# risc0/zeth

Hardware: AMD Instinct MI355X
Metric: segments/sec (higher is better)
Workload: dtype u32

## Files before the change

### zeth_amd/csrc/common.h

```cpp
#pragma once
#include <hip/hip_runtime.h>

#include <atomic>
#include <cstdarg>
#include <cstdio>
#include <cstdlib>
#include <cstring>
#include <map>
#include <string>
#include <vector>

#include "../../include/zkhal.h"
#include "fp.h"
#include "noise.h"

namespace zkh {

inline const char* make_err(const char* fmt, ...) {
    char buf[512];
    va_list ap;
    va_start(ap, fmt);
    vsnprintf(buf, sizeof buf, fmt, ap);
    va_end(ap);
    return strdup(buf);
}
#define ZKH_HIP(expr)                                                                               \
    do {                                                                                            \
        hipError_t _e = (expr);                                                                     \
        if (_e != hipSuccess) return zkh::make_err("%s failed: %s (%s:%d)", #expr, hipGetErrorString(_e), __FILE__, __LINE__); \
    } while (0)
#define ZKH_TRY(expr)                    \
    do {                                 \
        const char* _err = (expr);       \
        if (_err) return _err;           \
    } while (0)
#define ZKH_REQUIRE(cond, ...)                         \
    do {                                               \
        if (!(cond)) return zkh::make_err(__VA_ARGS__); \
    } while (0)

constexpr int ZKH_P2_PTAB = 414;
constexpr int TW_BITS = 12;
constexpr int TW_SIZE = 1 << TW_BITS;
constexpr int TW_HI_BITS = 14;
constexpr int TW_HI_SIZE = 1 << TW_HI_BITS;
constexpr int MAX_LOG_N = TW_BITS + TW_HI_BITS;
constexpr int LDS_TW_LOG = 12;

struct DeviceTables {
    uint32_t* rc;
    uint32_t* diag;
    uint32_t* tw_fwd_lo; uint32_t* tw_fwd_hi;
    uint32_t* tw_rev_lo; uint32_t* tw_rev_hi;
    uint32_t* tile_fwd;  uint32_t* tile_rev;
    uint32_t* layer_fwd; uint32_t* layer_rev;
    uint32_t* layer_fwd_lazy;
    uint32_t* shift_lo;  uint32_t* shift_hi;
};

struct ProfAgg { uint64_t calls = 0; double ms = 0; double bytes = 0; };
struct ProfPending { std::string name; hipEvent_t a, b; double bytes; };

}

struct zkh_alloc_t {
    void* ptr;
    size_t bytes;
    std::atomic<int> refs;
    bool owned;
    zkh_ctx* ctx;
    zkh_alloc_t(void* p, size_t b, int r, bool o, zkh_ctx* c) : ptr(p), bytes(b), refs(r), owned(o), ctx(c) {}
};

struct zkh_buf {
    zkh_alloc_t* a;
    size_t off, len;
    std::atomic<int> refs;
    zkh_buf(zkh_alloc_t* al, size_t o, size_t l, int r) : a(al), off(o), len(l), refs(r) {}
    uint32_t* ptr() const { return (uint32_t*)a->ptr + off; }
};

struct zkh_ctx {
    int device;
    hipStream_t stream;
    zkh::DeviceTables tab;
    uint32_t rou_fwd[28], rou_rev[28];
    uint32_t h_rc[24 * 29], h_diag[zkh::ZKH_P2_PTAB];
    std::multimap<size_t, void*> pool;
    size_t pool_bytes = 0, live_bytes = 0, peak_bytes = 0;
// ... 58 lines not shown
```

### zeth_amd/csrc/fp.h

```cpp
#pragma once
#include <stdint.h>

#if defined(__HIPCC__)
#include <hip/hip_runtime.h>
#define ZKH_HD __host__ __device__ __forceinline__
#else
#define ZKH_HD inline
#endif

namespace zkh {

constexpr uint32_t P = 2013265921u;
constexpr uint32_t PINV = 0x88000001u;
constexpr uint32_t NEG_PINV = 0x77ffffffu;
constexpr uint32_t R1 = 268435454u;
constexpr uint32_t R2 = 1172168163u;
constexpr uint32_t INVALID = 0xffffffffu;

struct Fp {
    uint32_t v;
    ZKH_HD Fp() : v(0) {}
    ZKH_HD explicit constexpr Fp(uint32_t raw, int) : v(raw) {}
    static ZKH_HD Fp raw(uint32_t r) { return Fp(r, 0); }
    static ZKH_HD Fp one() { return Fp(R1, 0); }
// ... 21 lines not shown
    return borrow ? t + P : t;
#endif
}
ZKH_HD uint32_t mont_reduce(uint64_t t) {
    const uint32_t m = (uint32_t)t * NEG_PINV;
    const uint64_t s = t + (uint64_t)m * P;
    return reduce_once((uint32_t)(s >> 32));
}
ZKH_HD int64_t mad_i64(int32_t a, int32_t b, int64_t acc) {
#if defined(__HIP_DEVICE_COMPILE__)
    int64_t d; uint64_t carry;
    asm("v_mad_i64_i32 %0, %1, %2, %3, %4" : "=v"(d), "=s"(carry) : "v"(a), "v"(b), "v"(acc));
    return d;
#else
    return (int64_t)((uint64_t)acc + (uint64_t)((int64_t)a * b));
#endif
}
ZKH_HD int64_t mad_i64_k(int32_t a, int32_t b_uniform, int64_t acc) {
#if defined(__HIP_DEVICE_COMPILE__)
    int64_t d; uint64_t carry;
    asm("v_mad_i64_i32 %0, %1, %2, %3, %4" : "=v"(d), "=s"(carry) : "v"(a), "s"(b_uniform), "v"(acc));
    return d;
#else
    return (int64_t)((uint64_t)acc + (uint64_t)((int64_t)a * b_uniform));
#endif
}
ZKH_HD int64_t mul_i64(int32_t a, int32_t b) {
#if defined(__HIP_DEVICE_COMPILE__)
    int64_t d; uint64_t carry;
    asm("v_mad_i64_i32 %0, %1, %2, %3, 0" : "=v"(d), "=s"(carry) : "v"(a), "v"(b));
    return d;
#else
    return (int64_t)a * b;
#endif
}
ZKH_HD int32_t smont_reduce(int64_t t) {
    const int32_t m = (int32_t)((uint32_t)t * NEG_PINV);
    return (int32_t)(mad_i64_k(m, (int32_t)P, t) >> 32);
}
ZKH_HD int32_t smont(int32_t a, int32_t b) {
    const int64_t t = (int64_t)a * b;
    const int32_t m = (int32_t)((uint32_t)t * NEG_PINV);
    const int64_t s = t + (int64_t)m * (int64_t)P;
    return (int32_t)(s >> 32);
}
ZKH_HD uint32_t canon(int32_t x) { const uint32_t u = (uint32_t)x, v = u + P; return v < u ? v : u; }
ZKH_HD int32_t center(uint32_t x) { return (int32_t)(x - (x > (P - 1) / 2 ? P : 0u)); }
ZKH_HD uint32_t mul_mod(uint32_t a, uint32_t b) { return mont_reduce((uint64_t)a * b); }

ZKH_HD Fp operator+(Fp a, Fp b) { return Fp::raw(add_mod(a.v, b.v)); }
ZKH_HD Fp operator-(Fp a, Fp b) { return Fp::raw(sub_mod(a.v, b.v)); }
ZKH_HD Fp operator*(Fp a, Fp b) { return Fp::raw(mul_mod(a.v, b.v)); }
ZKH_HD Fp operator-(Fp a) { return Fp::raw(a.v ? P - a.v : 0); }
ZKH_HD bool operator==(Fp a, Fp b) { return a.v == b.v; }
ZKH_HD Fp& operator+=(Fp& a, Fp b) { a = a + b; return a; }
ZKH_HD Fp& operator-=(Fp& a, Fp b) { a = a - b; return a; }
ZKH_HD Fp& operator*=(Fp& a, Fp b) { a = a * b; return a; }

ZKH_HD Fp fp_encode(uint32_t x) { return Fp::raw(mul_mod(R2, x % P)); }
ZKH_HD uint32_t fp_decode(Fp a) { return mul_mod(1u, a.v); }
ZKH_HD Fp fp_pow(Fp a, uint64_t e) {
    Fp r = Fp::one();
    while (e) { if (e & 1) r = r * a; a = a * a; e >>= 1; }
    return r;
}
ZKH_HD Fp fp_inv(Fp a) { return fp_pow(a, P - 2); }
// ... 81 lines not shown
```

### zeth_amd/csrc/hal.hip

```cpp
#include <algorithm>

#include "common.h"

#include <sys/random.h>
#include "poseidon2.h"
#include "ntt_lazy.h"
#include "../../include/zkh_poseidon2_consts.h"

using namespace zkh;

extern "C" void zkh_free_error(const char* e) { free((void*)e); }
#if ZKH_P2_CONSTS_ARE_PLACEHOLDER
extern "C" const char* zkh_version(void) { return "zkhal-mi355x 0.2.0 (gfx950; poseidon2_consts=placeholder)"; }
#elif ZKH_P2_CONSTS_ARE_DERIVED
extern "C" const char* zkh_version(void) { return "zkhal-mi355x 0.2.0 (gfx950; poseidon2_consts=derived)"; }
#else
extern "C" const char* zkh_version(void) { return "zkhal-mi355x 0.2.0 (gfx950; poseidon2_consts=upstream)"; }
#endif

namespace zkh {

const char* pool_alloc(zkh_ctx* c, size_t bytes, void** out) {
    bytes = (bytes + 255) & ~(size_t)255;
    if (bytes == 0) bytes = 256;
// ... 135 lines not shown
    if (const char* err = ctx_init_tables(c)) {
        zkh_ctx_destroy(c);
        return err;
    }
    *out = c;
    return nullptr;
}
static const char* ctx_init_tables(zkh_ctx* c) {
    Fp g = fp_encode(137);
    for (int k = 0; k <= 27; k++) {
        Fp w = fp_pow(g, 1ull << (27 - k));
        c->rou_fwd[k] = w.v;
        c->rou_rev[k] = fp_inv(w).v;
    }
    Fp wf = Fp::raw(c->rou_fwd[MAX_LOG_N]), wr = Fp::raw(c->rou_rev[MAX_LOG_N]);
    ZKH_TRY(upload(&c->tab.tw_fwd_lo, powers(wf, TW_SIZE)));
    ZKH_TRY(upload(&c->tab.tw_fwd_hi, powers(fp_pow(wf, TW_SIZE), TW_HI_SIZE)));
    ZKH_TRY(upload(&c->tab.tw_rev_lo, powers(wr, TW_SIZE)));
    ZKH_TRY(upload(&c->tab.tw_rev_hi, powers(fp_pow(wr, TW_SIZE), TW_HI_SIZE)));
    ZKH_TRY(upload(&c->tab.tile_fwd, powers(Fp::raw(c->rou_fwd[LDS_TW_LOG]), 1 << (LDS_TW_LOG - 1))));
    ZKH_TRY(upload(&c->tab.tile_rev, powers(Fp::raw(c->rou_rev[LDS_TW_LOG]), 1 << (LDS_TW_LOG - 1))));
    {
        std::vector<uint32_t> lf(1 << LDS_TW_LOG, R1), lr(1 << LDS_TW_LOG, R1);
        for (int j = 1; j <= LDS_TW_LOG; j++) {
            auto pf = powers(Fp::raw(c->rou_fwd[j]), (size_t)1 << (j - 1)), pr = powers(Fp::raw(c->rou_rev[j]), (size_t)1 << (j - 1));
            for (size_t e = 0; e < pf.size(); e++) { lf[((size_t)1 << (j - 1)) + e] = pf[e]; lr[((size_t)1 << (j - 1)) + e] = pr[e]; }
        }
        ZKH_TRY(upload(&c->tab.layer_fwd, lf));
        ZKH_TRY(upload(&c->tab.layer_rev, lr));
        static_assert(LAZY_TAB_LOG == LDS_TW_LOG, "the lazy table covers the per-layer tables");
        std::vector<uint32_t> lz(LAZY_TAB_WORDS);
        lazy_layer_table(lz.data(), lf.data());
        ZKH_TRY(upload(&c->tab.layer_fwd_lazy, lz));
    }
    Fp three = fp_encode(3);
    ZKH_TRY(upload(&c->tab.shift_lo, powers(three, TW_SIZE)));
    ZKH_TRY(upload(&c->tab.shift_hi, powers(fp_pow(three, TW_SIZE), TW_HI_SIZE)));
    ZKH_TRY(upload(&c->tab.rc, std::vector<uint32_t>(24 * 29)));
    ZKH_TRY(upload(&c->tab.diag, std::vector<uint32_t>(ZKH_P2_PTAB)));
    ZKH_TRY(zkh_poseidon2_set_constants(c, ZKH_P2_ROUND_CONSTANTS, ZKH_P2_M_INT_DIAG));
    ZKH_TRY(ntt_device_init(c));
    ZKH_HIP(hipMalloc((void**)&c->d_fail, 8));
    ZKH_HIP(hipMemsetAsync(c->d_fail, 0, 8, c->stream));
    ZKH_HIP(hipHostMalloc((void**)&c->h_fail, 8, hipHostMallocDefault));
    c->h_fail[0] = c->h_fail[1] = 0;
    return nullptr;
}
extern "C" const char* zkh_ctx_trim(zkh_ctx* c) {
    bind_thread(c);
    ZKH_HIP(hipStreamSynchronize(c->stream));
    for (auto& kv : c->pool) (void)hipFree(kv.second);
    c->pool.clear(); c->pool_bytes = 0;
    return nullptr;
}
extern "C" void zkh_ctx_memory(const zkh_ctx* c, size_t* live, size_t* cached, size_t* peak) {
    if (live) *live = c->live_bytes;
    if (cached) *cached = c->pool_bytes;
    if (peak) *peak = c->peak_bytes;
}
extern "C" void zkh_ctx_destroy(zkh_ctx* c) {
    if (!c) return;
    (void)hipSetDevice(c->device);
    (void)hipStreamSynchronize(c->stream);
    for (auto& kv : c->pool) (void)hipFree(kv.second);
    uint32_t* t[] = {c->tab.rc, c->tab.diag, c->tab.tw_fwd_lo, c->tab.tw_fwd_hi, c->tab.tw_rev_lo, c->tab.tw_rev_hi,
                     c->tab.tile_fwd, c->tab.tile_rev, c->tab.shift_lo, c->tab.shift_hi, c->tab.layer_fwd, c->tab.layer_rev, c->tab.layer_fwd_lazy};
// ... 396 lines not shown
```

### zeth_amd/csrc/ntt.hip

```cpp
#include "common.h"
#include "ntt_lazy.h"

using namespace zkh;

namespace {

constexpr int NTT_THREADS = 256;

struct PassParams {
    const uint32_t* in;
    uint32_t* out;
    size_t in_col_stride;
    size_t out_col_stride;
    uint32_t log_n;
    uint32_t L, R;
    uint32_t log_t;
    uint32_t expand_bits;
    uint32_t first_layer;
    uint32_t twiddle;
    uint32_t scale;
    uint32_t zk_shift;
    const uint32_t* tile_tw;
    const uint32_t* layer_tw;
    const uint32_t* tw_lo;
    const uint32_t* tw_hi;
    const uint32_t* sh_lo;
    const uint32_t* sh_hi;
    uint32_t tiles_per_col;
    uint32_t lazy;
    uint32_t lazy_comp;
    uint32_t shift16[16];
};

template <bool INVERSE>
__global__ __launch_bounds__(NTT_THREADS) void k_ntt_pass(PassParams p) {
    extern __shared__ __attribute__((aligned(16))) uint32_t tile[];
    const uint32_t T = 1u << p.log_t, rows = 1u << p.R, elems = rows << p.log_t;
    const uint32_t tid = threadIdx.x;
    const uint32_t tile_id = xcd_remap(blockIdx.x, p.tiles_per_col);
    const uint32_t col = blockIdx.y;
    const uint32_t ltiles = 1u << (p.L - p.log_t);
    const uint32_t a = tile_id >> (p.L - p.log_t), lt = tile_id & (ltiles - 1);
    const size_t base = ((size_t)a << (p.L + p.R)) + ((size_t)lt << p.log_t);
    const uint32_t l0 = lt << p.log_t;
    const uint32_t* in = p.in + (size_t)col * p.in_col_stride;
    uint32_t* out = p.out + (size_t)col * p.out_col_stride;
    const uint32_t tw_shift = MAX_LOG_N - (p.L + p.R);

    for (uint32_t e = tid; e < elems; e += NTT_THREADS) {
        const uint32_t m = e >> p.log_t, t = e & (T - 1);
        const size_t gi = base + ((size_t)m << p.L) + t;
        uint32_t v = in[gi >> p.expand_bits];
        if (!INVERSE && p.twiddle) {
            const uint32_t r = __brev(m) >> (32 - p.R);
            const uint32_t ex = ((l0 + t) * r) << tw_shift;
            const uint32_t w = mul_mod(p.tw_lo[ex & (TW_SIZE - 1)], p.tw_hi[ex >> TW_BITS]);
            v = mul_mod(v, w);
        }
        tile[e] = v;
    }
    __syncthreads();

    const uint32_t half_elems = elems >> 1;
    if (INVERSE) {
// ... 138 lines not shown
    const uint32_t mid = blockIdx.x;
    const uint32_t rmid = mid_bits ? __brev(mid) >> (32 - mid_bits) : 0;
    if (rmid < mid) return;
    uint32_t* col = io + (size_t)blockIdx.y * col_stride;
    const uint32_t H = 1u << BR_H;
    for (uint32_t e = threadIdx.x; e < H * H; e += blockDim.x) {
        const uint32_t hi = e >> BR_H, lo = e & (H - 1);
        ta[e] = col[((size_t)hi << (log_n - BR_H)) | ((size_t)mid << BR_H) | lo];
        if (rmid != mid) tb[e] = col[((size_t)hi << (log_n - BR_H)) | ((size_t)rmid << BR_H) | lo];
    }
    __syncthreads();
    for (uint32_t e = threadIdx.x; e < H * H; e += blockDim.x) {
        const uint32_t hi2 = e >> BR_H, lo2 = e & (H - 1);
        const uint32_t shi = __brev(lo2) >> (32 - BR_H), slo = __brev(hi2) >> (32 - BR_H);
        const uint32_t src = (shi << BR_H) | slo;
        col[((size_t)hi2 << (log_n - BR_H)) | ((size_t)rmid << BR_H) | lo2] = ta[src];
        if (rmid != mid) col[((size_t)hi2 << (log_n - BR_H)) | ((size_t)mid << BR_H) | lo2] = tb[src];
    }
}
__global__ void k_bit_reverse_small(uint32_t* io, uint32_t log_n, size_t count) {
    size_t g = (size_t)blockIdx.x * blockDim.x + threadIdx.x;
    size_t n = (size_t)1 << log_n;
    if (g >= n * count) return;
    uint32_t i = (uint32_t)(g & (n - 1));
    uint32_t r = log_n ? __brev(i) >> (32 - log_n) : 0;
    if (i < r) {
        uint32_t* col = io + (g - i);
        uint32_t x = col[i], y = col[r];
        col[i] = y; col[r] = x;
    }
}


template <int LOGR, bool INVERSE, bool BASE0, int J_LO, bool LAZY = false>
__device__ __forceinline__ void radix_layers(uint32_t (&v)[1 << LOGR], const uint32_t* __restrict__ ltab,
                                             const uint32_t base_low, const int first_b) {
    constexpr int N = 1 << LOGR;
    if (!INVERSE && LAZY) {
        lazy_layers<LOGR, BASE0, J_LO>(v, ltab, base_low, first_b);
    } else if (INVERSE) {
#pragma unroll
        for (int b = LOGR - 1; b >= 0; b--) {
            const uint32_t* tw = ltab + (1u << (J_LO + b - 1));
#pragma unroll
            for (int kk = 0; kk < (1 << b); kk++) {
                const bool unit = BASE0 && kk == 0;
                const uint32_t w = unit ? 0u : tw[base_low + ((uint32_t)kk << (J_LO - 1))];
#pragma unroll
                for (int hi = 0; hi < (N >> (b + 1)); hi++) {
                    const int k = (hi << (b + 1)) | kk;
                    const uint32_t x = v[k], y = v[k + (1 << b)];
                    v[k] = add_mod(x, y);
                    v[k + (1 << b)] = unit ? sub_mod(x, y) : mul_mod(x - y + P, w);
                }
            }
        }
    } else {
#pragma unroll
        for (int b = 0; b < LOGR; b++) {
            if (b < first_b) continue;
            const uint32_t* tw = ltab + (1u << (J_LO + b - 1));
#pragma unroll
            for (int kk = 0; kk < (1 << b); kk++) {
                const bool unit = BASE0 && kk == 0;
                const uint32_t w = unit ? 0u : tw[base_low + ((uint32_t)kk << (J_LO - 1))];
#pragma unroll
                for (int hi = 0; hi < (N >> (b + 1)); hi++) {
                    const int k = (hi << (b + 1)) | kk;
                    const uint32_t x = v[k], y = unit ? v[k + (1 << b)] : mul_mod(v[k + (1 << b)], w);
                    v[k] = add_mod(x, y);
                    v[k + (1 << b)] = sub_mod(x, y);
                }
            }
        }
    }
// ... 46 lines not shown
        if (p.expand_bits == 0) {
#pragma unroll
            for (int q = 0; q < 4; q++) {
                const uint4 w = ((const uint4*)(in + pos0))[q];
                v[4 * q] = w.x; v[4 * q + 1] = w.y; v[4 * q + 2] = w.z; v[4 * q + 3] = w.w;
            }
        } else if (p.expand_bits == 2) {
            const uint4 w = *(const uint4*)(in + (pos0 >> 2));
            v[0] = v[1] = v[2] = v[3] = w.x; v[4] = v[5] = v[6] = v[7] = w.y;
            v[8] = v[9] = v[10] = v[11] = w.z; v[12] = v[13] = v[14] = v[15] = w.w;
        } else {
#pragma unroll
            for (int k = 0; k < 16; k++) v[k] = in[(pos0 + k) >> p.expand_bits];
        }
        radix_layers<4, false, true, 1, LAZY>(v, ltab, 0, (int)p.expand_bits);
#pragma unroll
        for (int q = 0; q < 4; q++) ((uint4*)lds)[tid * 4 + q] = make_uint4(v[4 * q], v[4 * q + 1], v[4 * q + 2], v[4 * q + 3]);
        __syncthreads();
#pragma unroll
        for (int k = 0; k < 16; k++) v[k] = lds[hi * 256 + k * 16 + low];
        radix_layers<4, false, false, 5, LAZY>(v, ltab, low, 0);
#pragma unroll
        for (int k = 0; k < 16; k++) lds[hi * 256 + k * 16 + low] = v[k];
        __syncthreads();
#pragma unroll
        for (int k = 0; k < 16; k++) v[k] = lds[k * 256 + tid];
        radix_layers<4, false, false, 9, LAZY>(v, ltab, tid, 0);
#pragma unroll
        for (int k = 0; k < 16; k++) out[base + k * 256 + tid] = v[k];
    }
}

template <int RH, bool INVERSE, bool LAZY = false>
__global__ __launch_bounds__(1 << RH) void k_ntt_high(PassParams p) {
    constexpr int LT = 4;
    constexpr uint32_t TW = 1u << LT;
    extern __shared__ __attribute__((aligned(16))) uint32_t lds[];
    const uint32_t tid = threadIdx.x, t = tid & (TW - 1), g = tid >> LT;
    const uint32_t tile_id = xcd_remap(blockIdx.x, p.tiles_per_col), col = blockIdx.y;
    const uint32_t lt_bits = p.L - LT;
    const uint32_t a = tile_id >> lt_bits, lt = tile_id & ((1u << lt_bits) - 1);
    const size_t base = ((size_t)a << (p.L + RH)) + ((size_t)lt << LT);
    const uint32_t lcol = (lt << LT) + t;
    const uint32_t tw_shift = MAX_LOG_N - (p.L + RH);
    const char* in = (const char*)(p.in + (size_t)col * p.in_col_stride + base);
    char* out = (char*)(p.out + (size_t)col * p.out_col_stride + base);
    const uint32_t tb = t * 4u;
#define TILE_IN(row) (*(const uint32_t*)(in + ((((uint32_t)(row)) << (p.L + 2)) + tb)))
#define TILE_OUT(row) (*(uint32_t*)(out + ((((uint32_t)(row)) << (p.L + 2)) + tb)))
    const uint32_t* __restrict__ ltab = p.layer_tw;
    auto tmul = [](uint32_t x, uint32_t y) -> uint32_t {
        return (LAZY && !INVERSE) ? (uint32_t)smont((int32_t)x, (int32_t)y) : mul_mod(x, y);
    };
    auto root = [&](uint32_t e) -> uint32_t {
        const uint32_t ex = e << tw_shift;
        return tmul(p.tw_lo[ex & (TW_SIZE - 1)], p.tw_hi[ex >> TW_BITS]);
    };
    uint32_t tw[16];
    if (RH == 10) {
        uint32_t w0 = root(lcol * (__brev(g) >> 26));
        if (LAZY) w0 = tmul(w0, p.lazy_comp);
        const uint32_t u1 = root(lcol * 64u), v1 = root(lcol * 256u);
        const uint32_t u2 = tmul(u1, u1), u3 = tmul(u2, u1), v2 = tmul(v1, v1), v3 = tmul(v2, v1);
        const uint32_t wi[4] = {w0, tmul(w0, u2), tmul(w0, u1), tmul(w0, u3)};
#pragma unroll
        for (int i = 0; i < 4; i++) {
            tw[4 * i] = wi[i]; tw[4 * i + 1] = tmul(wi[i], v2); tw[4 * i + 2] = tmul(wi[i], v1); tw[4 * i + 3] = tmul(wi[i], v3);
        }
    } else {
        uint32_t w0 = root(lcol * (__brev(g) >> 28));
        if (LAZY) w0 = tmul(w0, p.lazy_comp);
        const uint32_t q1 = root(lcol * 16u);
        uint32_t qp[16];
        qp[0] = w0;
#pragma unroll
        for (int e = 1; e < 16; e++) qp[e] = tmul(qp[e - 1], q1);
#pragma unroll
        for (int k = 0; k < 16; k++) tw[k] = qp[__builtin_bitreverse8((unsigned char)k) >> 4];
    }
    uint32_t v[16];
    if (RH == 10) {
        const uint32_t hi = g >> 2, low = g & 3;
        if (INVERSE) {
#pragma unroll
            for (int k = 0; k < 16; k++) v[k] = TILE_IN(k * 64 + g);
            radix_layers<4, true, false, 7>(v, ltab, g, 0);
#pragma unroll
            for (int k = 0; k < 16; k++) lds[(k * 64 + g) * TW + t] = v[k];
            __syncthreads();
#pragma unroll
            for (int k = 0; k < 16; k++) v[k] = lds[(hi * 64 + k * 4 + low) * TW + t];
            radix_layers<4, true, false, 3>(v, ltab, low, 0);
#pragma unroll
            for (int k = 0; k < 16; k++) lds[(hi * 64 + k * 4 + low) * TW + t] = v[k];
            __syncthreads();
#pragma unroll
            for (int i = 0; i < 4; i++) {
                uint32_t u[4];
                const uint32_t m0 = (g * 4 + i) * 4;
#pragma unroll
                for (int k = 0; k < 4; k++) u[k] = lds[(m0 + k) * TW + t];
                radix_layers<2, true, true, 1>(u, ltab, 0, 0);
#pragma unroll
                for (int k = 0; k < 4; k++) {
                    uint32_t x = mul_mod(u[k], tw[4 * i + k]);
                    if (p.scale) x = mul_mod(x, p.scale);
                    TILE_OUT(m0 + k) = x;
                }
            }
        } else {
#pragma unroll
            for (int i = 0; i < 4; i++) {
                uint32_t u[4];
                const uint32_t m0 = (g * 4 + i) * 4;
#pragma unroll
                for (int k = 0; k < 4; k++) {
                    const uint32_t x = TILE_IN(m0 + k);
                    u[k] = LAZY ? (uint32_t)smont((int32_t)x, (int32_t)tw[4 * i + k]) : mul_mod(x, tw[4 * i + k]);
                }
                radix_layers<2, false, true, 1, LAZY>(u, ltab, 0, 0);
#pragma unroll
                for (int k = 0; k < 4; k++) lds[(m0 + k) * TW + t] = u[k];
            }
            __syncthreads();
#pragma unroll
            for (int k = 0; k < 16; k++) v[k] = lds[(hi * 64 + k * 4 + low) * TW + t];
            radix_layers<4, false, false, 3, LAZY>(v, ltab, low, 0);
#pragma unroll
            for (int k = 0; k < 16; k++) lds[(hi * 64 + k * 4 + low) * TW + t] = v[k];
            __syncthreads();
#pragma unroll
            for (int k = 0; k < 16; k++) v[k] = lds[(k * 64 + g) * TW + t];
            radix_layers<4, false, false, 7, LAZY>(v, ltab, g, 0);
#pragma unroll
            for (int k = 0; k < 16; k++) TILE_OUT(k * 64 + g) = LAZY ? canon((int32_t)v[k]) : v[k];
        }
    } else {
        if (INVERSE) {
#pragma unroll
            for (int k = 0; k < 16; k++) v[k] = TILE_IN(k * 16 + g);
            radix_layers<4, true, false, 5>(v, ltab, g, 0);
#pragma unroll
            for (int k = 0; k < 16; k++) lds[(k * 16 + g) * TW + t] = v[k];
            __syncthreads();
#pragma unroll
            for (int k = 0; k < 16; k++) v[k] = lds[(g * 16 + k) * TW + t];
            radix_layers<4, true, true, 1>(v, ltab, 0, 0);
#pragma unroll
            for (int k = 0; k < 16; k++) {
                uint32_t x = mul_mod(v[k], tw[k]);
                if (p.scale) x = mul_mod(x, p.scale);
                TILE_OUT(g * 16 + k) = x;
            }
        } else {
#pragma unroll
            for (int k = 0; k < 16; k++) {
                const uint32_t x = TILE_IN(g * 16 + k);
                v[k] = LAZY ? (uint32_t)smont((int32_t)x, (int32_t)tw[k]) : mul_mod(x, tw[k]);
            }
            radix_layers<4, false, true, 1, LAZY>(v, ltab, 0, 0);
#pragma unroll
            for (int k = 0; k < 16; k++) lds[(g * 16 + k) * TW + t] = v[k];
            __syncthreads();
#pragma unroll
            for (int k = 0; k < 16; k++) v[k] = lds[(k * 16 + g) * TW + t];
            radix_layers<4, false, false, 5, LAZY>(v, ltab, g, 0);
#pragma unroll
            for (int k = 0; k < 16; k++) TILE_OUT(k * 16 + g) = LAZY ? canon((int32_t)v[k]) : v[k];
        }
    }
}
#undef TILE_IN
#undef TILE_OUT

struct Pass { uint32_t L, R; };
std::vector<Pass> plan_passes(uint32_t log_n) {
    std::vector<Pass> v;
    if (log_n <= 12) { v.push_back({0, log_n}); return v; }
    if (log_n < 18) {
        const uint32_t low = (log_n + 1) / 2;
        v.push_back({0, low});
        v.push_back({low, log_n - low});
        return v;
    }
    const uint32_t rem = log_n - 12;
    v.push_back({0, 12});
    if (rem == 8 || rem == 10 || rem <= 7) v.push_back({12, rem});
    else if (rem == 9) { v.push_back({12, 8}); v.push_back({20, 1}); }
    else if (rem == 11 || rem == 12) { v.push_back({12, 8}); v.push_back({20, rem - 8}); }
    else { v.push_back({12, 10}); v.push_back({22, rem - 10}); }
    return v;
}

const char* run_transform(zkh_ctx* c, bool inverse, const uint32_t* in, size_t in_col_stride, uint32_t* out,
                          size_t out_col_stride, uint32_t log_n, size_t count, uint32_t expand_bits, bool zk, const char* name) {
    ZKH_REQUIRE(log_n <= (uint32_t)MAX_LOG_N, "%s: transform size 2^%u exceeds the supported 2^%d", name, log_n, MAX_LOG_N);
    ZKH_REQUIRE(count <= 65535, "%s: too many columns (%zu)", name, count);
    std::vector<Pass> passes = plan_passes(log_n);
    const size_t n = (size_t)1 << log_n;
    Fp ninv = fp_inv(fp_encode((uint32_t)(n % P)));
    const size_t npass = passes.size();
    const bool lazy = !inverse && npass == 2 && passes[0].R == 12 && (passes[1].R == 8 || passes[1].R == 10) && expand_bits <= 4;
    const uint32_t lazy_reds = lazy ? lazy_reductions(4, expand_bits) + 2 * lazy_reductions(4, 0) + lazy_reductions(passes[1].R, 0) : 0;
    const uint32_t lazy_comp = lazy ? fp_pow(Fp::raw(R2), lazy_reds).v : 0;
    for (size_t pi = 0; pi < npass; pi++) {
        const Pass ps = inverse ? passes[npass - 1 - pi] : passes[pi];
        PassParams p{};
        const bool first = pi == 0, last = pi + 1 == npass;
        p.in = first ? in : out;
        p.in_col_stride = first ? in_col_stride : out_col_stride;
        p.out = out; p.out_col_stride = out_col_stride;
        p.log_n = log_n; p.L = ps.L; p.R = ps.R;
        const bool reg_high = ps.L >= 4 && (ps.R == 8 || ps.R == 10);
        p.log_t = ps.L == 0 ? 0 : (ps.L < 4 ? ps.L : 4);
        if (ps.L != 0 && !reg_high && ps.R < 12) p.log_t = std::max<uint32_t>(p.log_t, std::min<uint32_t>(ps.L, 12 - ps.R));
        while (p.R + p.log_t > 14 && p.log_t > 0) p.log_t--;
        p.expand_bits = (!inverse && first) ? expand_bits : 0;
        p.first_layer = (!inverse && first) ? expand_bits + 1 : 1;
        p.twiddle = ps.L != 0;
        p.scale = (inverse && last) ? ninv.v : 0;
        p.zk_shift = (inverse && last && zk) ? 1 : 0;
        p.lazy = lazy; p.lazy_comp = lazy_comp;
        p.tile_tw = inverse ? c->tab.tile_rev : c->tab.tile_fwd;
        p.layer_tw = inverse ? c->tab.layer_rev : (lazy ? c->tab.layer_fwd_lazy : c->tab.layer_fwd);
        p.tw_lo = inverse ? c->tab.tw_rev_lo : c->tab.tw_fwd_lo;
        p.tw_hi = inverse ? c->tab.tw_rev_hi : c->tab.tw_fwd_hi;
        p.sh_lo = c->tab.shift_lo; p.sh_hi = c->tab.shift_hi;
        if (p.zk_shift && log_n >= 4) {
            const Fp three = fp_encode(3);
            for (uint32_t k = 0; k < 16; k++)
                p.shift16[k] = (ninv * fp_pow(three, (uint64_t)(bitrev32(k) >> 28) << (log_n - 4))).v;
        }
        p.tiles_per_col = (uint32_t)(n >> (p.R + p.log_t));
        const size_t lds = ((size_t)4 << (p.R + p.log_t));
        dim3 grid(p.tiles_per_col, (unsigned)count);
        const double alg_bytes = pi == 0 ? 4.0 * count * (double)(((size_t)1 << log_n) >> expand_bits) + 4.0 * count * (double)n : 0.0;
        const bool scale_here = p.scale != 0;
        const bool k_low = ps.L == 0 && ps.R == 12 && p.expand_bits <= 4;
        const bool k_h10 = !k_low && ps.L >= 4 && p.log_t == 4 && ps.R == 10 && !(scale_here && p.zk_shift);
        const bool k_h8 = !k_low && !k_h10 && ps.L >= 4 && p.log_t == 4 && ps.R == 8 && !(scale_here && p.zk_shift);
        const bool k_top = !k_low && !k_h10 && !k_h8 && ps.L >= 12 && ps.L + ps.R == log_n && ps.R >= 1 && ps.R <= 4 && p.twiddle &&
                           p.expand_bits == 0 && p.first_layer == 1 && !scale_here && !p.zk_shift;
        const std::string pname = std::string(name) + (k_low ? ":k_ntt_low12" : k_h10 ? ":k_ntt_high10" : k_h8 ? ":k_ntt_high8" : k_top ? ":k_ntt_top" : ":k_ntt_pass");
        ProfScope prof(c, pname.c_str(), alg_bytes);
        if (ps.L == 0 && ps.R == 12 && p.expand_bits <= 4) {
            if (inverse) k_ntt_low12<true><<<grid, 256, 0, c->stream>>>(p);
            else if (lazy) k_ntt_low12<false, true><<<grid, 256, 0, c->stream>>>(p);
            else k_ntt_low12<false><<<grid, 256, 0, c->stream>>>(p);
        } else if (ps.L >= 4 && p.log_t == 4 && ps.R == 10 && !(scale_here && p.zk_shift)) {
            if (inverse) k_ntt_high<10, true><<<grid, 1024, lds, c->stream>>>(p);
            else if (lazy) k_ntt_high<10, false, true><<<grid, 1024, lds, c->stream>>>(p);
            else k_ntt_high<10, false><<<grid, 1024, lds, c->stream>>>(p);
        } else if (ps.L >= 4 && p.log_t == 4 && ps.R == 8 && !(scale_here && p.zk_shift)) {
            if (inverse) k_ntt_high<8, true><<<grid, 256, lds, c->stream>>>(p);
            else if (lazy) k_ntt_high<8, false, true><<<grid, 256, lds, c->stream>>>(p);
            else k_ntt_high<8, false><<<grid, 256, lds, c->stream>>>(p);
        } else if (k_top) {
            const dim3 tg((unsigned)(((size_t)1 << ps.L) >> 10), (unsigned)count);
            switch (ps.R * 2 + (inverse ? 1 : 0)) {
            case 2: k_ntt_top<1, false><<<tg, 256, 0, c->stream>>>(p); break;
            case 3: k_ntt_top<1, true><<<tg, 256, 0, c->stream>>>(p); break;
            case 4: k_ntt_top<2, false><<<tg, 256, 0, c->stream>>>(p); break;
            case 5: k_ntt_top<2, true><<<tg, 256, 0, c->stream>>>(p); break;
            case 6: k_ntt_top<3, false><<<tg, 256, 0, c->stream>>>(p); break;
            case 7: k_ntt_top<3, true><<<tg, 256, 0, c->stream>>>(p); break;
            case 8: k_ntt_top<4, false><<<tg, 256, 0, c->stream>>>(p); break;
            default: k_ntt_top<4, true><<<tg, 256, 0, c->stream>>>(p); break;
            }
        } else if (inverse) k_ntt_pass<true><<<grid, NTT_THREADS, lds, c->stream>>>(p);
        else k_ntt_pass<false><<<grid, NTT_THREADS, lds, c->stream>>>(p);
        ZKH_TRY(last_launch_error(name));
    }
    return nullptr;
}

}

const char* zkh::ntt_device_init(zkh_ctx* c) {
    bind_thread(c);
    ZKH_HIP(hipFuncSetAttribute((const void*)k_ntt_high<10, true>, hipFuncAttributeMaxDynamicSharedMemorySize, 65536));
    ZKH_HIP(hipFuncSetAttribute((const void*)k_ntt_high<10, false>, hipFuncAttributeMaxDynamicSharedMemorySize, 65536));
    ZKH_HIP(hipFuncSetAttribute((const void*)k_ntt_high<10, false, true>, hipFuncAttributeMaxDynamicSharedMemorySize, 65536));
    return nullptr;
}

static const char* interpolate_impl(zkh_ctx* c, zkh_buf* io, size_t count, bool zk, const char* name) {
    ZKH_REQUIRE(count && io->len % count == 0, "%s: size %zu not a multiple of count %zu", name, io->len, count);
    const size_t n = io->len / count;
    const uint32_t log_n = log2_ceil(n);
    ZKH_REQUIRE(((size_t)1 << log_n) == n, "%s: column length %zu is not a power of two", name, n);
    return run_transform(c, true, io->ptr(), n, io->ptr(), n, log_n, count, 0, zk, name);
}
extern "C" const char* zkh_batch_interpolate_ntt(zkh_ctx* c, zkh_buf* io, size_t count) {
    return interpolate_impl(c, io, count, false, "batch_interpolate_ntt");
}
extern "C" const char* zkh_batch_interpolate_ntt_zk_shift(zkh_ctx* c, zkh_buf* io, size_t count) {
    return interpolate_impl(c, io, count, true, "batch_interpolate_ntt_zk_shift");
}
extern "C" const char* zkh_batch_interpolate_ntt_from(zkh_ctx* c, zkh_buf* out, const zkh_buf* in, size_t count, int zk_shift) {
    ZKH_REQUIRE(count && in->len % count == 0 && out->len == in->len, "batch_interpolate_ntt_from: shape mismatch");
    const size_t n = in->len / count;
    const uint32_t log_n = log2_ceil(n);
    ZKH_REQUIRE(((size_t)1 << log_n) == n, "batch_interpolate_ntt_from: column length %zu is not a power of two", n);
    return run_transform(c, true, in->ptr(), n, out->ptr(), n, log_n, count, 0, zk_shift != 0, "batch_interpolate_ntt_from");
}
extern "C" const char* zkh_batch_expand_into_evaluate_ntt(zkh_ctx* c, zkh_buf* out, const zkh_buf* in, size_t count,
                                                          size_t expand_bits) {
    ZKH_REQUIRE(count && out->len % count == 0 && in->len % count == 0, "batch_expand_into_evaluate_ntt: sizes not multiples of count");
    const size_t n_out = out->len / count, n_in = in->len / count;
    const uint32_t log_n = log2_ceil(n_out);
    ZKH_REQUIRE(((size_t)1 << log_n) == n_out && (n_in << expand_bits) == n_out,
                "batch_expand_into_evaluate_ntt: out column %zu != in column %zu << %zu", n_out, n_in, expand_bits);
    ZKH_REQUIRE(expand_bits <= log_n, "batch_expand_into_evaluate_ntt: expand_bits too large");
    if (expand_bits == log_n) {
        return make_err("batch_expand_into_evaluate_ntt: expand_bits == log2(size) unsupported");
// ... 28 lines not shown
```

### zeth_amd/csrc/ntt_lazy.h

```cpp
#pragma once
#include "fp.h"

#ifndef ZKH_LAZY_SUM
#define ZKH_LAZY_SUM(t) ((void)0)
#endif

namespace zkh {

constexpr int LAZY_TAB_LOG = 12;
constexpr uint32_t LAZY_TAB_MONT = 1u << LAZY_TAB_LOG;
constexpr uint32_t LAZY_TAB_WORDS = 2u << LAZY_TAB_LOG;

inline void lazy_layer_table(uint32_t* out, const uint32_t* layer_fwd) {
    for (uint32_t i = 0; i < LAZY_TAB_MONT; i++) {
        out[i] = (uint32_t)center(mont_reduce((uint64_t)layer_fwd[i]));
        out[LAZY_TAB_MONT + i] = (uint32_t)center(layer_fwd[i]);
    }
}

template <bool UNIFORM>
ZKH_HD int64_t lazy_mad(int32_t a, int32_t w, int64_t acc) {
    if constexpr (UNIFORM) return mad_i64_k(a, w, acc);
    else return mad_i64(a, w, acc);
}
// ... 35 lines not shown
    constexpr int N = 1 << LOGR;
#pragma unroll
    for (int b = 0; b < LOGR; b += 2) {
        const uint32_t* twa = ltab + (1u << (J_LO + b - 1));
        const uint32_t* twb = ltab + LAZY_TAB_MONT + (1u << (J_LO + b));
        if (b >= first_b) {
#pragma unroll
            for (int kk = 0; kk < (1 << b); kk++) {
                const uint32_t e = base_low + ((uint32_t)kk << (J_LO - 1));
                const int32_t wa = (BASE0 && kk == 0) ? 1 : (int32_t)twa[e];
                const int32_t wb0 = (BASE0 && kk == 0) ? (int32_t)R1 : (int32_t)twb[e];
                const int32_t wb1 = (int32_t)twb[e + ((1u << b) << (J_LO - 1))];
#pragma unroll
                for (int hi = 0; hi < (N >> (b + 2)); hi++) {
                    const int k = (hi << (b + 2)) | kk;
                    lazy_pair<BASE0>(v[k], v[k + (1 << b)], v[k + (2 << b)], v[k + (3 << b)], wa, wb0, wb1);
                }
            }
        } else if (b + 1 >= first_b) {
            const uint32_t* tw1 = ltab + (1u << (J_LO + b));
#pragma unroll
            for (int kk = 0; kk < (2 << b); kk++) {
                const int32_t w = (BASE0 && kk == 0) ? 1 : (int32_t)tw1[base_low + ((uint32_t)kk << (J_LO - 1))];
#pragma unroll
                for (int hi = 0; hi < (N >> (b + 2)); hi++) {
                    const int k = (hi << (b + 2)) | kk;
                    lazy_single<BASE0>(v[k], v[k + (2 << b)], w);
                }
            }
        }
    }
}

}
```

Measured before the change: 44.43.

## Add lazy signed-Montgomery inverse tail for strided high NTT pass

```diff
diff --git a/zeth_amd/csrc/common.h b/zeth_amd/csrc/common.h
--- a/zeth_amd/csrc/common.h
+++ b/zeth_amd/csrc/common.h
@@ -55,6 +55,7 @@
     uint32_t* tile_fwd;  uint32_t* tile_rev;
     uint32_t* layer_fwd; uint32_t* layer_rev;
     uint32_t* layer_fwd_lazy;
+    int32_t lazy_inv_a = 0, lazy_inv_b = 0;
     uint32_t* shift_lo;  uint32_t* shift_hi;
 };
 
diff --git a/zeth_amd/csrc/fp.h b/zeth_amd/csrc/fp.h
--- a/zeth_amd/csrc/fp.h
+++ b/zeth_amd/csrc/fp.h
@@ -77,6 +77,15 @@
     return d;
 #else
     return (int64_t)a * b;
+#endif
+}
+ZKH_HD int64_t mul_i64_k(int32_t a, int32_t b_uniform) {
+#if defined(__HIP_DEVICE_COMPILE__)
+    int64_t d; uint64_t carry;
+    asm("v_mad_i64_i32 %0, %1, %2, %3, 0" : "=v"(d), "=s"(carry) : "v"(a), "s"(b_uniform));
+    return d;
+#else
+    return (int64_t)a * b_uniform;
 #endif
 }
 ZKH_HD int32_t smont_reduce(int64_t t) {
diff --git a/zeth_amd/csrc/hal.hip b/zeth_amd/csrc/hal.hip
--- a/zeth_amd/csrc/hal.hip
+++ b/zeth_amd/csrc/hal.hip
@@ -191,6 +191,8 @@
         std::vector<uint32_t> lz(LAZY_TAB_WORDS);
         lazy_layer_table(lz.data(), lf.data());
         ZKH_TRY(upload(&c->tab.layer_fwd_lazy, lz));
+        ZKH_REQUIRE(lazy_inv_short_pair(fp_decode(Fp::raw(lr[3])), &c->tab.lazy_inv_a, &c->tab.lazy_inv_b),
+                    "no short pair a^2 + b^2 = P for the inverse NTT's strided pass");
     }
     Fp three = fp_encode(3);
     ZKH_TRY(upload(&c->tab.shift_lo, powers(three, TW_SIZE)));
diff --git a/zeth_amd/csrc/ntt.hip b/zeth_amd/csrc/ntt.hip
--- a/zeth_amd/csrc/ntt.hip
+++ b/zeth_amd/csrc/ntt.hip
@@ -30,6 +30,7 @@
     uint32_t lazy;
     uint32_t lazy_comp;
     uint32_t shift16[16];
+    int32_t lazy_a, lazy_b;
 };
 
 template <bool INVERSE>
@@ -234,7 +235,7 @@
 }
 
 
-template <int LOGR, bool INVERSE, bool BASE0, int J_LO, bool LAZY = false>
+template <int LOGR, bool INVERSE, bool BASE0, int J_LO, bool LAZY = false, int LAST_B = 0>
 __device__ __forceinline__ void radix_layers(uint32_t (&v)[1 << LOGR], const uint32_t* __restrict__ ltab,
                                              const uint32_t base_low, const int first_b) {
     constexpr int N = 1 << LOGR;
@@ -242,7 +243,7 @@
         lazy_layers<LOGR, BASE0, J_LO>(v, ltab, base_low, first_b);
     } else if (INVERSE) {
 #pragma unroll
-        for (int b = LOGR - 1; b >= 0; b--) {
+        for (int b = LOGR - 1; b >= LAST_B; b--) {
             const uint32_t* tw = ltab + (1u << (J_LO + b - 1));
 #pragma unroll
             for (int kk = 0; kk < (1 << b); kk++) {
@@ -355,7 +356,7 @@
 }
 
 template <int RH, bool INVERSE, bool LAZY = false>
-__global__ __launch_bounds__(1 << RH) void k_ntt_high(PassParams p) {
+__global__ __launch_bounds__(1 << RH, INVERSE && LAZY ? (RH == 10 ? 8 : 7) : 0) void k_ntt_high(PassParams p) {
     constexpr int LT = 4;
     constexpr uint32_t TW = 1u << LT;
     extern __shared__ __attribute__((aligned(16))) uint32_t lds[];
@@ -373,34 +374,37 @@
 #define TILE_OUT(row) (*(uint32_t*)(out + ((((uint32_t)(row)) << (p.L + 2)) + tb)))
     const uint32_t* __restrict__ ltab = p.layer_tw;
     auto tmul = [](uint32_t x, uint32_t y) -> uint32_t {
-        return (LAZY && !INVERSE) ? (uint32_t)smont((int32_t)x, (int32_t)y) : mul_mod(x, y);
+        return LAZY ? (uint32_t)smont((int32_t)x, (int32_t)y) : mul_mod(x, y);
     };
     auto root = [&](uint32_t e) -> uint32_t {
         const uint32_t ex = e << tw_shift;
         return tmul(p.tw_lo[ex & (TW_SIZE - 1)], p.tw_hi[ex >> TW_BITS]);
     };
     uint32_t tw[16];
-    if (RH == 10) {
-        uint32_t w0 = root(lcol * (__brev(g) >> 26));
-        if (LAZY) w0 = tmul(w0, p.lazy_comp);
-        const uint32_t u1 = root(lcol * 64u), v1 = root(lcol * 256u);
-        const uint32_t u2 = tmul(u1, u1), u3 = tmul(u2, u1), v2 = tmul(v1, v1), v3 = tmul(v2, v1);
-        const uint32_t wi[4] = {w0, tmul(w0, u2), tmul(w0, u1), tmul(w0, u3)};
-#pragma unroll
-        for (int i = 0; i < 4; i++) {
-            tw[4 * i] = wi[i]; tw[4 * i + 1] = tmul(wi[i], v2); tw[4 * i + 2] = tmul(wi[i], v1); tw[4 * i + 3] = tmul(wi[i], v3);
-        }
-    } else {
-        uint32_t w0 = root(lcol * (__brev(g) >> 28));
-        if (LAZY) w0 = tmul(w0, p.lazy_comp);
-        const uint32_t q1 = root(lcol * 16u);
-        uint32_t qp[16];
-        qp[0] = w0;
-#pragma unroll
-        for (int e = 1; e < 16; e++) qp[e] = tmul(qp[e - 1], q1);
-#pragma unroll
-        for (int k = 0; k < 16; k++) tw[k] = qp[__builtin_bitreverse8((unsigned char)k) >> 4];
-    }
+    constexpr bool TW_LATE = INVERSE && LAZY;
+#define FOUR_STEP_TW() \
+    if (RH == 10) {                                                                                                               \
+        uint32_t w0 = root(lcol * (__brev(g) >> 26));                                                                             \
+        if (LAZY) w0 = tmul(w0, p.lazy_comp);                                                                                     \
+        const uint32_t u1 = root(lcol * 64u), v1 = root(lcol * 256u);                                                             \
+        const uint32_t u2 = tmul(u1, u1), u3 = tmul(u2, u1), v2 = tmul(v1, v1), v3 = tmul(v2, v1);                                \
+        const uint32_t wi[4] = {w0, tmul(w0, u2), tmul(w0, u1), tmul(w0, u3)};                                                    \
+        _Pragma("unroll")                                                                                                         \
+        for (int i = 0; i < 4; i++) {                                                                                             \
+            tw[4 * i] = wi[i]; tw[4 * i + 1] = tmul(wi[i], v2); tw[4 * i + 2] = tmul(wi[i], v1); tw[4 * i + 3] = tmul(wi[i], v3); \
+        }                                                                                                                         \
+    } else {                                                                                                                      \
+        uint32_t w0 = root(lcol * (__brev(g) >> 28));                                                                             \
+        if (LAZY) w0 = tmul(w0, p.lazy_comp);                                                                                     \
+        const uint32_t q1 = root(lcol * 16u);                                                                                     \
+        uint32_t qp[16];                                                                                                          \
+        qp[0] = w0;                                                                                                               \
+        _Pragma("unroll")                                                                                                         \
+        for (int e = 1; e < 16; e++) qp[e] = tmul(qp[e - 1], q1);                                                                 \
+        _Pragma("unroll")                                                                                                         \
+        for (int k = 0; k < 16; k++) tw[k] = qp[__builtin_bitreverse8((unsigned char)k) >> 4];                                    \
+    }
+    if (!TW_LATE) { FOUR_STEP_TW() }
     uint32_t v[16];
     if (RH == 10) {
         const uint32_t hi = g >> 2, low = g & 3;
@@ -417,18 +421,25 @@
 #pragma unroll
             for (int k = 0; k < 16; k++) lds[(hi * 64 + k * 4 + low) * TW + t] = v[k];
             __syncthreads();
+            if (TW_LATE) { auto make_tw = [&]() { FOUR_STEP_TW() }; make_tw(); }
 #pragma unroll
             for (int i = 0; i < 4; i++) {
                 uint32_t u[4];
                 const uint32_t m0 = (g * 4 + i) * 4;
 #pragma unroll
                 for (int k = 0; k < 4; k++) u[k] = lds[(m0 + k) * TW + t];
-                radix_layers<2, true, true, 1>(u, ltab, 0, 0);
-#pragma unroll
-                for (int k = 0; k < 4; k++) {
-                    uint32_t x = mul_mod(u[k], tw[4 * i + k]);
-                    if (p.scale) x = mul_mod(x, p.scale);
-                    TILE_OUT(m0 + k) = x;
+                if (LAZY) {
+                    lazy_inv_tail<2>(u, p.lazy_a, p.lazy_b, tw + 4 * i);
+#pragma unroll
+                    for (int k = 0; k < 4; k++) TILE_OUT(m0 + k) = canon((int32_t)u[k]);
+                } else {
+                    radix_layers<2, true, true, 1>(u, ltab, 0, 0);
+#pragma unroll
+                    for (int k = 0; k < 4; k++) {
+                        uint32_t x = mul_mod(u[k], tw[4 * i + k]);
+                        if (p.scale) x = mul_mod(x, p.scale);
+                        TILE_OUT(m0 + k) = x;
+                    }
                 }
             }
         } else {
@@ -468,12 +479,20 @@
             __syncthreads();
 #pragma unroll
             for (int k = 0; k < 16; k++) v[k] = lds[(g * 16 + k) * TW + t];
-            radix_layers<4, true, true, 1>(v, ltab, 0, 0);
-#pragma unroll
-            for (int k = 0; k < 16; k++) {
-                uint32_t x = mul_mod(v[k], tw[k]);
-                if (p.scale) x = mul_mod(x, p.scale);
-                TILE_OUT(g * 16 + k) = x;
+            if (TW_LATE) { auto make_tw = [&]() { FOUR_STEP_TW() }; make_tw(); }
+            if (LAZY) {
+                radix_layers<4, true, true, 1, false, 2>(v, ltab, 0, 0);
+                lazy_inv_tail<4>(v, p.lazy_a, p.lazy_b, tw);
+#pragma unroll
+                for (int k = 0; k < 16; k++) TILE_OUT(g * 16 + k) = canon((int32_t)v[k]);
+            } else {
+                radix_layers<4, true, true, 1>(v, ltab, 0, 0);
+#pragma unroll
+                for (int k = 0; k < 16; k++) {
+                    uint32_t x = mul_mod(v[k], tw[k]);
+                    if (p.scale) x = mul_mod(x, p.scale);
+                    TILE_OUT(g * 16 + k) = x;
+                }
             }
         } else {
 #pragma unroll
@@ -493,6 +512,7 @@
         }
     }
 }
+#undef FOUR_STEP_TW
 #undef TILE_IN
 #undef TILE_OUT
 
@@ -524,6 +544,7 @@
     Fp ninv = fp_inv(fp_encode((uint32_t)(n % P)));
     const size_t npass = passes.size();
     const bool lazy = !inverse && npass == 2 && passes[0].R == 12 && (passes[1].R == 8 || passes[1].R == 10) && expand_bits <= 4;
+    const bool lazy_inv = inverse && npass == 2 && passes[0].R == 12 && (passes[1].R == 8 || passes[1].R == 10);
     const uint32_t lazy_reds = lazy ? lazy_reductions(4, expand_bits) + 2 * lazy_reductions(4, 0) + lazy_reductions(passes[1].R, 0) : 0;
     const uint32_t lazy_comp = lazy ? fp_pow(Fp::raw(R2), lazy_reds).v : 0;
     for (size_t pi = 0; pi < npass; pi++) {
@@ -544,6 +565,10 @@
         p.scale = (inverse && last) ? ninv.v : 0;
         p.zk_shift = (inverse && last && zk) ? 1 : 0;
         p.lazy = lazy; p.lazy_comp = lazy_comp;
+        if (lazy_inv && ps.L != 0) {
+            p.lazy = 1; p.lazy_a = c->tab.lazy_inv_a; p.lazy_b = c->tab.lazy_inv_b;
+            p.lazy_comp = (uint32_t)lazy_inv_comp(c->tab.lazy_inv_a, p.scale);
+        }
         p.tile_tw = inverse ? c->tab.tile_rev : c->tab.tile_fwd;
         p.layer_tw = inverse ? c->tab.layer_rev : (lazy ? c->tab.layer_fwd_lazy : c->tab.layer_fwd);
         p.tw_lo = inverse ? c->tab.tw_rev_lo : c->tab.tw_fwd_lo;
@@ -571,11 +596,13 @@
             else if (lazy) k_ntt_low12<false, true><<<grid, 256, 0, c->stream>>>(p);
             else k_ntt_low12<false><<<grid, 256, 0, c->stream>>>(p);
         } else if (ps.L >= 4 && p.log_t == 4 && ps.R == 10 && !(scale_here && p.zk_shift)) {
-            if (inverse) k_ntt_high<10, true><<<grid, 1024, lds, c->stream>>>(p);
+            if (lazy_inv) k_ntt_high<10, true, true><<<grid, 1024, lds, c->stream>>>(p);
+            else if (inverse) k_ntt_high<10, true><<<grid, 1024, lds, c->stream>>>(p);
             else if (lazy) k_ntt_high<10, false, true><<<grid, 1024, lds, c->stream>>>(p);
             else k_ntt_high<10, false><<<grid, 1024, lds, c->stream>>>(p);
         } else if (ps.L >= 4 && p.log_t == 4 && ps.R == 8 && !(scale_here && p.zk_shift)) {
-            if (inverse) k_ntt_high<8, true><<<grid, 256, lds, c->stream>>>(p);
+            if (lazy_inv) k_ntt_high<8, true, true><<<grid, 256, lds, c->stream>>>(p);
+            else if (inverse) k_ntt_high<8, true><<<grid, 256, lds, c->stream>>>(p);
             else if (lazy) k_ntt_high<8, false, true><<<grid, 256, lds, c->stream>>>(p);
             else k_ntt_high<8, false><<<grid, 256, lds, c->stream>>>(p);
         } else if (k_top) {
@@ -604,6 +631,7 @@
     ZKH_HIP(hipFuncSetAttribute((const void*)k_ntt_high<10, true>, hipFuncAttributeMaxDynamicSharedMemorySize, 65536));
     ZKH_HIP(hipFuncSetAttribute((const void*)k_ntt_high<10, false>, hipFuncAttributeMaxDynamicSharedMemorySize, 65536));
     ZKH_HIP(hipFuncSetAttribute((const void*)k_ntt_high<10, false, true>, hipFuncAttributeMaxDynamicSharedMemorySize, 65536));
+    ZKH_HIP(hipFuncSetAttribute((const void*)k_ntt_high<10, true, true>, hipFuncAttributeMaxDynamicSharedMemorySize, 65536));
     return nullptr;
 }
 
diff --git a/zeth_amd/csrc/ntt_lazy.h b/zeth_amd/csrc/ntt_lazy.h
--- a/zeth_amd/csrc/ntt_lazy.h
+++ b/zeth_amd/csrc/ntt_lazy.h
@@ -91,4 +91,53 @@
     }
 }
 
+
+inline bool lazy_inv_short_pair(uint32_t iota, int32_t* a, int32_t* b) {
+    for (uint64_t x = 1; x * x < P; x++) {
+        const uint64_t r = P - x * x;
+        uint64_t y = (uint64_t)__builtin_sqrt((double)r);
+        while (y * y > r) y--;
+        while ((y + 1) * (y + 1) <= r) y++;
+        if (y * y != r) continue;
+        const uint64_t ix = (uint64_t)iota * x % P;
+        if (ix != y && ix != P - y) return false;
+        *a = (int32_t)x;
+        *b = ix == y ? (int32_t)y : -(int32_t)y;
+        return true;
+    }
+    return false;
 }
+inline int32_t lazy_inv_comp(int32_t a, uint32_t scale) {
+    const Fp k = fp_inv(Fp::raw((uint32_t)a));
+    return center(scale ? (k * Fp::raw(scale)).v : k.v);
+}
+
+template <bool UNIFORM>
+ZKH_HD int64_t lazy_mul(int32_t a, int32_t w) {
+    if constexpr (UNIFORM) return mul_i64_k(a, w);
+    else return mul_i64(a, w);
+}
+template <bool UNIFORM>
+ZKH_HD void lazy_inv_bfly(uint32_t& v0, uint32_t& v1, int32_t ws, int32_t wd, int32_t nwd) {
+    const int32_t x = (int32_t)v0, y = (int32_t)v1;
+    v0 = (uint32_t)lazy_reduce(lazy_mad<UNIFORM>(y, ws, lazy_mul<UNIFORM>(x, ws)));
+    v1 = (uint32_t)lazy_reduce(lazy_mad<UNIFORM>(y, nwd, lazy_mul<UNIFORM>(x, wd)));
+}
+template <int LOGR>
+ZKH_HD void lazy_inv_tail(uint32_t (&v)[1 << LOGR], const int32_t a, const int32_t b, const uint32_t* c) {
+    constexpr int N = 1 << LOGR;
+    static_assert(LOGR >= 2, "the short pair needs the layer with twiddle i");
+    const int32_t na = -a, nb = -b;
+#pragma unroll
+    for (int k = 0; k < N; k += 4) {
+        lazy_inv_bfly<true>(v[k], v[k + 2], a, a, na);
+        lazy_inv_bfly<true>(v[k + 1], v[k + 3], a, b, nb);
+    }
+#pragma unroll
+    for (int k = 0; k < N; k += 2) {
+        const int32_t c0 = (int32_t)c[k], c1 = (int32_t)c[k + 1];
+        lazy_inv_bfly<false>(v[k], v[k + 1], c0, c1, -c1);
+    }
+}
+
+}
```

Result: no change. 44.37 (-0.1%).
